# KevinLADLee/RoboRTS-Edu-SLAM

Measured on AMD Instinct MI355X. Metric: candidate-pose scorings/sec (1081-beam scan, 2000×2000 grid) at 1/2/4/8 GPUs, higher is better.
Workload: dtype f64; 1 GPU; config2: 1081-beam scans vs 2000x2000 @5cm fp32 grid, full 3-level coarse->fine->super-fine (sim-YAML windows 5070+1331+189 candidates/scan); levels=headline, scans_per_gpu=4096, parallelism=replicas x1 (scan-sharded, no collective)

## Files before the change

roborts-edu-slam_amd/csrc/csm_api.cpp:

```cpp
#include "csm_source_digest.h"
#include "csm_host.hpp"
#include "libm_sincos.hpp"

using namespace csmh;

extern "C" {

int csm_abi_version(void) { return CSM_ABI_VERSION; }

const char* csm_build_digest(void) { return CSM_SOURCE_DIGEST; }

int csm_create(int device, csm_ctx** out) {
  const char* lr = std::getenv("LOCAL_RANK");
  const char* lw = std::getenv("LOCAL_WORLD_SIZE");
  const int world = lw ? std::max(1, std::atoi(lw)) : 1;
  const int rank = (lr && world > 1) ? std::min(std::max(0, std::atoi(lr)), world - 1) : 0;
  return create_context(device, rank, world, out);
}

int csm_get_host_plan(csm_ctx* c, csm_host_plan* out) {
  if (!c || !out) return CSM_ERR_INVALID_ARG;
  *out = c->host_plan;
  return CSM_OK;
}
// ... 20 lines not shown
  if (const char* env = std::getenv("CSM_HOST_THREADS")) {
    const int v = std::atoi(env);
    if (v > 0) c->host_plan.threads = v;
  }
  c->host_threads = c->host_plan.threads;
  if (const char* env = std::getenv("CSM_FIRST_WINDOWS")) c->first_windows = c->first_windows_submit = std::max(0, std::atoi(env));
  if (const char* env = std::getenv("CSM_FIRST_WINDOWS_SUBMIT")) c->first_windows_submit = std::max(0, std::atoi(env));
  if (const char* env = std::getenv("CSM_SPLIT_HANDOFF_MIN")) c->split_handoff_min = std::max(2, std::atoi(env));
  if (const char* env = std::getenv("CSM_DEFER_HANDOFF")) c->defer_last_handoff = std::atoi(env) != 0;
  if (const char* env = std::getenv("CSM_HOST_SIGNAL")) c->host_signal = std::atoi(env) != 0;
  if (const char* env = std::getenv("CSM_FINISH")) {
    c->device_finish = std::strcmp(env, "host") != 0;
    c->fast_finish = std::strcmp(env, "exact") != 0;
  }
  if (const char* env = std::getenv("CSM_KERNEL")) {
    c->row_kernel = std::strcmp(env, "v2") != 0;
    c->box_kernel = std::strcmp(env, "v6") == 0 || std::strcmp(env, "v7") == 0;
    c->box_kernel = c->box_kernel || std::strcmp(env, "v8") == 0;
    c->phase_kernel = std::strcmp(env, "v7") == 0 || std::strcmp(env, "v8") == 0;
    c->tiny_kernel = std::strcmp(env, "v8") == 0;
    c->pair_kernel = false;
  }
  if (const char* env = std::getenv("CSM_PHASE_STRIPS")) c->phase_strips = std::atoi(env) != 0;
  if (const char* env = std::getenv("CSM_PHASE_MARGIN_LOG2"))
    c->phase_margin_log2 = std::max(2, std::min(std::atoi(env), 20));
  if (const char* env = std::getenv("CSM_PIPELINE")) {
    const int v = std::atoi(env);
    c->pipeline_min = v > 0 ? v : INT32_MAX;
  }
  if (const char* env = std::getenv("CSM_PIPELINE_PARTS"))
    c->pipeline_parts = std::max(2, std::min(std::atoi(env), csm_ctx::kMaxParts));
  if (const char* env = std::getenv("CSM_SKIP_DEAD_LISTS")) c->skip_dead_lists = std::atoi(env) != 0;
  if (const char* env = std::getenv("CSM_SMALL")) c->small_path = std::atoi(env) != 0;
  if (const char* env = std::getenv("CSM_LIST_REDUCE_MIN")) c->list_reduce_min = std::max<long long>(0, std::atoll(env));
  if (const char* env = std::getenv("CSM_STATS_DUMP")) c->stats_dump = std::atoi(env) != 0;
  if (const char* env = std::getenv("CSM_SCORE_MARKER")) c->score_marker = std::atoi(env) != 0;
  if (const char* env = std::getenv("CSM_DEVICE_TRIG")) c->device_trig = std::atoi(env) != 0;
#ifdef CSM_DEBUG_FIN
  c->debug_fin = true;
#endif
  if (c->each_slot([](LaunchSlot& s) { return s.create_sync_events(); }) != hipSuccess ||
      c->ev_pts.create(hipEventDisableTiming) != hipSuccess || c->ev_pack.create(hipEventDisableTiming) != hipSuccess ||
      c->x_stream.create(hipStreamNonBlocking) != hipSuccess) {
    delete c;
    return CSM_ERR_HIP;
  }
// ... 269 lines not shown
```

roborts-edu-slam_amd/csrc/csm_box.hip:

```cpp
#include <hip/hip_runtime.h>

#include <cstdint>
#include <cstdlib>

#include "csm_internal.hpp"
#include "csm_score_sink.hpp"

namespace csm {
namespace {

typedef int32_t v4i __attribute__((ext_vector_type(4)));

constexpr double kBoxMargin = 0x1p-20;

#ifndef CSM_RUN_SEG
#define CSM_RUN_SEG 1152
#endif
constexpr int kRunSeg = CSM_RUN_SEG;
#ifndef CSM_BOX_PF
#define CSM_BOX_PF 6
#endif
constexpr int kPF = CSM_BOX_PF;
#ifndef CSM_PAIR_ILP
#define CSM_PAIR_ILP 1
// ... 25 lines not shown
    const double tx = lx + hx;
    const double ty = ly + hy;
    const double fx = __builtin_amdgcn_fract(tx);
    const double fy = __builtin_amdgcn_fract(ty);
    const bool clean = tx >= 0.0 && ty >= 0.0 && fx >= kBoxMargin && fx <= 1.0 - kBoxMargin &&
                       fy >= kBoxMargin && fy <= 1.0 - kBoxMargin;
    const double lim = (double)(pad - nspan) - kBoxMargin;
    far = nspan > 0 && (tx <= lim || ty <= lim);
    ix0 = clean ? (int)tx : 0;
    iy0 = clean ? (int)ty : 0;
    return clean;
  }
  template <bool STRIP = false>
  __device__ __forceinline__ int offsets(const double2 p, int cb, uint64_t& slow) const {
    double lx, ly;
    int ix0, iy0;
    bool far;
    const bool clean = box_test(p, lx, ly, ix0, iy0, far);
    const bool live = cb + lane < n_used;
    const uint64_t rej = __builtin_amdgcn_ballot_w64(live && !clean && !far);
    if (rej) slow |= 1ull << min(cb >> 6, 63);
    int o;
    if (STRIP) {
      constexpr int S = kStripShift, LS = S == 4 ? 2 : 0;
      const int c = (-(ix0 >> LS)) & (kStripCopies - 1);
      const int xs = (ix0 & ~(S - 1)) + S * c;
      o = (int)(__umul24((uint32_t)c, (uint32_t)copy_bytes >> 4) << 4) +
          (int)__umul24((uint32_t)(xs >> 4), (uint32_t)strip_bytes) + iy0 * 16 + (ix0 & (S - 1));
    } else {
      o = iy0 * pitch4 + (ix0 << cell_shift);
    }
    return (live && clean && ix0 < sx + pad && iy0 < sy + pad) ? o : zero_off;
  }
  __device__ __forceinline__ double2 point(int cb) const {
    const uint32_t i = (uint32_t)min(cb + lane, n_used - 1);
    return *reinterpret_cast<const double2*>(reinterpret_cast<const char*>(P) + __umul24(i, step16));
  }

  template <int PF = kPF, typename CT = int32_t, bool STRIP = false, bool ILP = false>
  __device__ __forceinline__ int build_runs(int s0, int s1, int32_t* run_off, CT* run_cnt, int scratch,
                                            uint64_t& slow) const {
    int nruns = 0;
    double2 pq[PF];
#pragma unroll
    for (int u = 0; u < PF; ++u) {
      pq[u] = point(s0 + 64 * u);
      __builtin_amdgcn_sched_barrier(0);
    }
    for (int cb0 = s0; cb0 < s1; cb0 += 64 * PF) {
      int offv[PF];
      if constexpr (ILP) {
// ... 199 lines not shown
#ifdef CSM_BOX_TRACE
constexpr int kBoxTraceWaves = 4096;
__device__ unsigned long long g_box_trace[kBoxTraceWaves][12];
__device__ int g_box_trace_n;
#define BOX_STAMP() ((unsigned long long)__builtin_amdgcn_s_memtime())
#endif

constexpr int kPairPD = 2;
#ifndef CSM_PAIR_SEG
#define CSM_PAIR_SEG 576
#endif
constexpr int kPairSeg = CSM_PAIR_SEG;
static_assert(kPairSeg % 64 == 0 && (kPairSeg + 128) * 4 >= 16 * 16 * 8,
              "whole 64-beam chunks; the sums' transpose (16 x 16 int64) reuses the run list");

#ifndef CSM_PAIR_WAVES
#define CSM_PAIR_WAVES 0
#endif
#if CSM_PAIR_WAVES > 0
#define CSM_PAIR_BOUNDS __launch_bounds__(64, CSM_PAIR_WAVES)
#else
#define CSM_PAIR_BOUNDS __launch_bounds__(64)
#endif
template <int B>
__device__ __forceinline__ uint32_t byte_x8(uint32_t w) {
  static_assert(B >= 0 && B < 4, "a byte of a dword");
  uint32_t r;
  if constexpr (B == 0)
    asm("v_lshlrev_b32_sdwa %0, 3, %1 dst_sel:DWORD dst_unused:UNUSED_PAD src0_sel:DWORD src1_sel:BYTE_0"
        : "=v"(r) : "v"(w));
  else if constexpr (B == 1)
    asm("v_lshlrev_b32_sdwa %0, 3, %1 dst_sel:DWORD dst_unused:UNUSED_PAD src0_sel:DWORD src1_sel:BYTE_1"
        : "=v"(r) : "v"(w));
  else if constexpr (B == 2)
    asm("v_lshlrev_b32_sdwa %0, 3, %1 dst_sel:DWORD dst_unused:UNUSED_PAD src0_sel:DWORD src1_sel:BYTE_2"
        : "=v"(r) : "v"(w));
  else
    asm("v_lshlrev_b32_sdwa %0, 3, %1 dst_sel:DWORD dst_unused:UNUSED_PAD src0_sel:DWORD src1_sel:BYTE_3"
        : "=v"(r) : "v"(w));
  return r;
}

constexpr int kPairNoRunBeams = 128;

template <int NS, bool BEST, bool NORUN = false>
__global__ CSM_PAIR_BOUNDS void score_box_pair_kernel(LevelWork L, const ScanWork* __restrict__ scans,
                                                            const double2* __restrict__ pts,
                                                            const AngleEntry* __restrict__ angles,
                                                            double* __restrict__ out,
                                                            BestPartial* __restrict__ partials) {
  static_assert(NS >= 1 && NS <= kPalMaxSpace, "corner phase (<= 3) + NS cells within one 16-byte row piece");
  static_assert(kPairPD == 2, "a slot's step: one ds_read_b128 of pair offsets, one u16 of counts");
#ifdef CSM_BOX_TRACE
  unsigned long long tr[12] = {BOX_STAMP(), 0, 0, 0, 0, 0, 0, 0, 0, 0, 0, 0};
  unsigned long long tq = 0;
#endif
  const int bid = dev::xcd_remap(blockIdx.x, gridDim.x);
  dev::clear_word(L);
  const int win = bid / L.n_angles;
  const int a = bid - win * L.n_angles;
  const ScanWork S = scans[win];
  const AngleEntry ae = angles[S.angle_off + a];
  const int lane = threadIdx.x;
  const int k = lane & 15, slot = lane >> 4;
// ... 300 lines not shown
```

roborts-edu-slam_amd/csrc/csm_device.hpp:

```cpp
#pragma once

#include <hip/hip_runtime.h>

#include "csm_internal.hpp"

namespace csm {
namespace dev {

__device__ __forceinline__ void clear_word(int32_t* word, int32_t tag) {
  if (word && blockIdx.x == 0 && threadIdx.x == 0)
    __hip_atomic_store(reinterpret_cast<uint64_t*>(word), (uint64_t)(uint32_t)tag << 32, __ATOMIC_RELAXED,
                       __HIP_MEMORY_SCOPE_AGENT);
}
__device__ __forceinline__ void clear_word(const LevelWork& L) { clear_word(L.clear_word, L.clear_tag); }

__device__ __forceinline__ int xcd_remap(int orig, int nwg) {
  const int xcd = orig & 7;
  const int q = nwg >> 3, r = nwg & 7;
  const int base = (xcd < r) ? xcd * (q + 1) : r * (q + 1) + (xcd - r) * q;
  return base + (orig >> 3);
}

__device__ __forceinline__ double penalized(const LevelWork& L, const ScanWork& S, double acc, double x,
                                           double y, double angle) {
// ... 14 lines not shown
    }
  }
  return score;
}

__device__ __forceinline__ bool better(double s, int64_t f, double bs, int64_t bf) {
  return (s > bs) || (s == bs && f < bf);
}

__device__ __forceinline__ __amdgpu_buffer_rsrc_t uniform_rsrc(const void* p, int bytes) {
  const uint32_t lo = __builtin_amdgcn_readfirstlane((uint32_t)(uintptr_t)p);
  const uint32_t hi = __builtin_amdgcn_readfirstlane((uint32_t)((uintptr_t)p >> 32));
  return __builtin_amdgcn_make_buffer_rsrc((void*)(((uint64_t)hi << 32) | lo), (short)0, bytes, 0x00020000);
}

__device__ __forceinline__ void buffer_load_lds16(__amdgpu_buffer_rsrc_t rsrc,
                                                  __attribute__((address_space(3))) int32_t* lds,
                                                  int voffset) {
#if defined(__HIP_DEVICE_COMPILE__)
  __builtin_amdgcn_raw_ptr_buffer_load_lds(rsrc, lds, 16, voffset, 0, 0, 0);
#endif
}

__device__ __forceinline__ double bcast_lane(double v, int l) {
  const uint64_t u = __builtin_bit_cast(uint64_t, v);
  const uint32_t lo = __builtin_amdgcn_readlane((uint32_t)u, l);
  const uint32_t hi = __builtin_amdgcn_readlane((uint32_t)(u >> 32), l);
  return __builtin_bit_cast(double, ((uint64_t)hi << 32) | lo);
}

template <bool ROWS32>
__device__ __forceinline__ uint64_t swap_sum_u64(uint64_t u) {
  const uint32_t lo = (uint32_t)u, hi = (uint32_t)(u >> 32);
  if constexpr (ROWS32) {
    const auto l = __builtin_amdgcn_permlane32_swap(lo, lo, false, false);
    const auto h = __builtin_amdgcn_permlane32_swap(hi, hi, false, false);
    return (((uint64_t)h[0] << 32) | l[0]) + (((uint64_t)h[1] << 32) | l[1]);
  } else {
    const auto l = __builtin_amdgcn_permlane16_swap(lo, lo, false, false);
    const auto h = __builtin_amdgcn_permlane16_swap(hi, hi, false, false);
    return (((uint64_t)h[0] << 32) | l[0]) + (((uint64_t)h[1] << 32) | l[1]);
  }
}
template <int CTRL>
__device__ __forceinline__ uint64_t dpp_u64(uint64_t u) {
  const uint32_t lo = (uint32_t)__builtin_amdgcn_mov_dpp((int)(uint32_t)u, CTRL, 0xF, 0xF, false);
// ... 36 lines not shown
```

roborts-edu-slam_amd/csrc/csm_host.hpp:

```cpp
#pragma once

#include "csm.h"
#include "csm_internal.hpp"
#include "csm_finish_rules.hpp"
#include "csm_gridmap.h"
#include "csm_gridmap_internal.hpp"
#include "csm_resources.hpp"
#include "host_math.hpp"
#include "csm_pyramid.hpp"
#include "csm_search_match.hpp"
#include "csm_level_decision.hpp"

#include <algorithm>
#include <atomic>
#include <chrono>
#include <condition_variable>
#include <functional>
#include <memory>
#include <cfloat>
#include <cmath>
#include <cstdio>
#include <cstdlib>
#include <cstring>
#include <mutex>
// ... 355 lines not shown
  bool staging_dirty = false;
  csm_gridmap* reader_map = nullptr;
  csmh::HostBuf h_pts;
  csmh::Event ev_pts;
  bool ev_pts_used = false;
  bool host_signal = true;
  double t_call = 0.0, t_exit = 0.0;
  bool device_finish = true;
  bool fast_finish = true;
  int device_finish_min = 1;
  bool row_kernel = true;
  bool phase_kernel = true;
  bool tiny_kernel = true;
  int phase_margin_log2 = 20;
  csmh::DevBuf pal_grid, pal_vals, pal_scratch;
  csmh::DevBuf pal_strips;
  bool pal_strips_ok = false;
  bool pair_kernel = true;
  csmh::DevBuf istrips;
  uint64_t istrips_gen = 0;
  const int32_t* istrips_src = nullptr;
  bool istrips_ok = false;
  bool phase_strips = true;
  int32_t pal_n = 0;
  uint64_t pal_gen = 0;
  const int32_t* pal_src = nullptr;
  bool box_kernel = true;
  csmh::DevBuf split_slab, split_arrive, small_dev;
  csmh::HostBuf h_small_in, h_small_out;
  uint32_t flag_seq = 0;
  bool small_path = true;
  int small_max_windows = 32;
  int split_target_blocks = 512;
  int fast_wide_windows = 0;
  csmh::HostBuf h_pack;
  csmh::Event ev_pack;
  bool ev_pack_used = false;
  std::vector<double> pts_host;
  csmh::DevBuf d_updates;

  static constexpr int kParkedGrids = 3;
  csmh::GridState parked[kParkedGrids];
  uint64_t grid_clock = 0;
  void swap_grid(csmh::GridState& g) {
    std::swap(static_cast<csmh::GridState&>(*this), g);
    grid_gen = ++gen_clock;
// ... 235 lines not shown
```

roborts-edu-slam_amd/csrc/csm_launch.cpp:

```cpp
#include "csm_host.hpp"
#include "libm_sincos_table.hpp"

namespace csmh {

int window_dims(const csm_param& P, Dims& d) {
  if (!(P.search_angle_resolution > 0.0) || !(P.search_space_resolution > 0.0) ||
      !(P.search_angle_offset >= 0.0) || !(P.search_space_size >= 0.0))
    return CSM_ERR_INVALID_ARG;
  const double half = (P.search_angle_offset * 2) / 2;
  const double na = std::floor(half * 2 / P.search_angle_resolution) + 1;
  const double ns = round_half_away(P.search_space_size / P.search_space_resolution) + 1;
  if (!(na >= 1.0 && na < 1e7 && ns >= 1.0 && ns < 1e7)) return CSM_ERR_INVALID_ARG;
  d.n_angles = (int32_t)na;
  d.n_space = (int32_t)ns;
  d.n_cand = (int64_t)d.n_angles * d.n_space * d.n_space;
  return CSM_OK;
}

bool beam_rule(int n, int use_point_size, int& step, int& use, int& n_used) {
  use = use_point_size;
  if (n < 2 * use) {
    use = n;
    step = 1;
  } else {
// ... 391 lines not shown
constexpr bool kTailFinish = CSM_TAIL_FINISH != 0;

struct Launch {
  csm_ctx* c;
  const csm_param& P;
  const Dims& D;
  const Geometry& G;
  const std::vector<WindowPlan>& plans;
  const AngleEntry* angles;
  size_t n_angle_entries;
  Finish mode;
  int skip_lists;
  WinSpan sp;
  int nw, w0, w1;
  bool whole;
  double f;
  LevelSummary S{};
  LevelDecision dec{};
  LaunchShape shape{};
  csm::PhaseTable PT{};
  bool sig = false;
  int64_t stride = 0;
  LevelWork L{};
  csm::FinishArgs SA{};
  csm::FinishOut* sig_out = nullptr;
  int32_t* d_done = nullptr;
  const int32_t* flags_h = nullptr;
  int n_flags = 0;
  hipStream_t done_stream = nullptr;
  int nr() const { return w1 - w0; }
  bool time_fin() const { return c->profiling && !c->profile_first_level; }
  int validate(), decide(), level_work(const std::vector<int64_t>& pt_offsets, const std::vector<int32_t>& grid_index);
  int stage_signalled(), stage_tail(), send_inputs(), scoring();
  int launch_finish_timed(const csm::FinishArgs& A, csm::FinishOut* out, hipStream_t fs, bool fast_done);
  int finish_scores_to_host(), finish_signalled(), finish_device(), finish_best(BestPartial* best_out);
  void fill_pending(const char* kname, PendingRun& p);
};

int Launch::validate() {
  if (!whole) {
    bool ok = mode == Finish::kDevice && (sp.score || sp.finish) && 0 <= w0 && w0 < w1 && w1 <= nw &&
              n_angle_entries == (size_t)nw * (size_t)D.n_angles && sp.level;
    for (int w = w0; ok && w < w1; ++w) ok = plans[(size_t)w].angle_off == (int64_t)w * D.n_angles;
    if (!ok) return c->fail(CSM_ERR_INVALID_ARG, "run_windows: bad window span");
  }
  const int st = ensure_int_grid(c);
// ... 18 lines not shown
  K.int_grid = c->int_ok;
  K.tail_finish = kTailFinish && sig;
  K.box = c->box_kernel && f == 1.0 && csm::box_supported(D.n_space) && pad_ok;
  K.phase = use_int && c->phase_kernel && f < 1.0 && phase_table(f, D.n_space, c->phase_margin_log2, PT) &&
            csm::phase_supported(D.n_space, PT.cells, PT.nq) && pad_ok;
  K.tiny = c->tiny_kernel && f < 1.0 && csm::tiny_supported(D.n_space, f) && pad_ok && gridi_cells * 4 < INT32_MAX;
  dec = level_decide(S, K, w0, w1);
  if (!dec.valid) return c->fail(CSM_ERR_INVALID_ARG, "run_windows: bad window span");
  ShapeFacts F;
  F.best = mode == Finish::kBest;
  if (use_int && c->row_kernel && D.n_space <= 64) {
    const double span = (double)(D.n_space - 1) * f;
    F.rows_sq = csm::rows_pick_sq(D.n_space, (int)std::floor(span * (1.0 + 1e-9) + 1e-9) + 2);
    if (c->info.size_x < 4 * F.rows_sq) F.rows_sq = 0;
  }
  int st;
  if (dec.box && c->pair_kernel && csm::box_pair_supported(D.n_space)) {
    if ((st = ensure_palette(c)) != CSM_OK) return st;
    F.pair_ok = c->pal_n > 0 && gridi_cells <= INT32_MAX && c->pal_strips_ok;
  }
  const int64_t tile_n = (D.n_space + 15) / 16;
  F.tiled_ok = c->box_kernel && f == 1.0 && pad_ok && (int64_t)nw * tile_n * tile_n * D.n_angles <= INT32_MAX;
  if (dec.phase && c->phase_strips && (st = ensure_istrips(c)) != CSM_OK) return st;
  shape = launch_shape(dec, D.n_angles, D.n_space, F);
  if (shape.bps * nr() > INT32_MAX) return c->fail(CSM_ERR_UNSUPPORTED, "window too large for one launch");
  stride = score_stride(c, D, mode);
  return CSM_OK;
}

int Launch::level_work(const std::vector<int64_t>& pt_offsets, const std::vector<int32_t>& grid_index) {
  const hipError_t e = c->h_sw.ensure((size_t)nw * sizeof(ScanWork));
  if (e != hipSuccess) return c->hip_fail(e, "hipHostMalloc(scans)");
  ScanWork* sw = (ScanWork*)c->h_sw.p;
  if (sp.score && !(sp.sw_ready && sp.sw_stride == stride && (const void*)sp.sw_ready == (const void*)sw))
    fill_scan_work(D, plans, pt_offsets, grid_index, sw, (size_t)w0, (size_t)w1, stride);
  L = make_level_work(c, P, D, G, nr(), dec.use_int);
  const bool tiled = shape.kernel == ScoreKernel::kBoxTiled;
  L.blocks_per_scan = tiled ? D.n_angles : (int32_t)shape.bps;
  L.max_n_used = dec.max_n_used;
  L.tile_n = tiled ? shape.ktiles : 0;
  if (shape.kernel == ScoreKernel::kBoxPair) {
    const csm::StripGeom SG = csm::strip_geom(c->info.size_x, c->info.size_y);
    L.pal_n = c->pal_n;
    L.pal_grid = (const uint8_t*)c->pal_grid.p;
    L.pal_vals = (const int32_t*)c->pal_vals.p;
    L.pal_stride = (int64_t)c->pitch * (c->info.size_y + csm::kGridiPadRows);
    L.pal_strips = (const uint8_t*)c->pal_strips.p;
    L.strip_bytes = (int32_t)SG.strip_bytes;
    L.strip_copy_bytes = (int32_t)SG.copy_bytes;
    L.strip_grid_bytes = SG.grid_bytes;
  }
  if (shape.kernel == ScoreKernel::kPhase && c->phase_strips && c->istrips_ok) {
    const csm::StripGeom SG = csm::istrip_geom(c->info.size_x, c->info.size_y);
    L.istrips = (const int32_t*)c->istrips.p;
    L.istrip_bytes = (int32_t)SG.strip_bytes;
    L.istrip_copy_bytes = (int32_t)SG.copy_bytes;
    L.istrip_grid_bytes = SG.grid_bytes;
  }
  L.n_cols = (int32_t)shape.n_cols;
  L.ktiles = shape.ktiles;
  L.col_blocks = (int32_t)shape.col_blocks;
  return CSM_OK;
}

// ... 252 lines not shown
    if (fst != CSM_OK) return fst;
  }
  const double tp1 = c->profiling ? now_ms() : 0.0;
  if (c->profiling) c->account("host:launch:flush_events", (float)(tp1 - tp0), 0.0, 0.0);
  int st;
  hipError_t e;
  if ((st = X.validate()) != CSM_OK) return st;
  if (X.whole && mode != Finish::kBest && c->int_ok && X.S.in_range && small_launch(c, D, nw))
    return run_windows_small(c, P, D, G, plans, pt_offsets, angles, n_angle_entries, grid_index,
                             mode == Finish::kDevice, pend, skip_lists);
  if ((st = X.decide()) != CSM_OK) return st;
  if ((st = X.level_work(pt_offsets, grid_index)) != CSM_OK) return st;
  if (X.sig && (st = X.stage_signalled()) != CSM_OK) return st;
  if (X.dec.tail && (st = X.stage_tail()) != CSM_OK) return st;
  if ((e = c->scans.ensure((size_t)nw * sizeof(ScanWork))) != hipSuccess) return c->hip_fail(e, "hipMalloc(scans)");
  if ((e = c->angles.ensure(n_angle_entries * sizeof(AngleEntry))) != hipSuccess) return c->hip_fail(e, "hipMalloc(angles)");
  const double tl0 = c->profiling ? now_ms() : 0.0;
  if (c->profiling) c->account("host:launch:prep", (float)(tl0 - tp1), 0.0, 0.0);
  if (sp.score && (st = X.send_inputs()) != CSM_OK) return st;
  char kname[48];
  score_kernel_name(X.shape, kname, sizeof(kname));
  const double tl1 = c->profiling ? now_ms() : 0.0;
  if ((st = X.scoring()) != CSM_OK) return st;
  if (c->profiling && mode != Finish::kBest) {
    c->account("host:launch:inputs", (float)(tl1 - tl0), 0.0, 0.0);
    c->account("host:launch:score", (float)(now_ms() - tl1), 0.0, 0.0);
  }
  if (!sp.finish) return CSM_OK;
  const double tl2 = (c->profiling && mode != Finish::kBest) ? now_ms() : 0.0;
  X.done_stream = c->d2h;
  st = mode == Finish::kBest ? X.finish_best(best_out)
       : mode == Finish::kScoresToHost ? X.finish_scores_to_host()
       : X.sig ? X.finish_signalled()
               : X.finish_device();
  if (st != CSM_OK) return st;
  PendingRun local;
  PendingRun& p = pend ? *pend : local;
  X.fill_pending(kname, p);
  if ((e = hipEventRecord(c->ev_done, X.done_stream)) != hipSuccess) return c->hip_fail(e, "hipEventRecord");
  if (c->profiling && tl2 > 0.0) c->account("host:launch:finish", (float)(now_ms() - tl2), 0.0, 0.0);
  if (c->profiling && X.sig) {
    char nm[48];
    std::snprintf(nm, sizeof(nm), "finish:%s<%lld>", X.dec.tail ? "fused" : "separate", (long long)D.n_cand);
    c->account(nm, 0.f, 0.0, (double)nw);
  }
  return pend ? CSM_OK : wait_run(c, p);
// ... 122 lines not shown
```

roborts-edu-slam_amd/csrc/csm_phase.hip:

```cpp
#include <hip/hip_runtime.h>

#include <cstdint>

#include "csm_internal.hpp"
#include "csm_score_sink.hpp"

namespace csm {
namespace {

#ifndef CSM_PHASE_SEG
#define CSM_PHASE_SEG 576
#endif
constexpr int kSeg = CSM_PHASE_SEG;
constexpr int kEntG = 31;
static_assert(kEntG * ((1LL << 26) - 1) < 2147483647LL, "a lane's int32 partial");
constexpr int kChunks = kSeg / 64;
#ifndef CSM_PHASE_DEPTH
#define CSM_PHASE_DEPTH 4
#endif
constexpr int kD = CSM_PHASE_DEPTH;
static_assert(kD <= 32, "int32 partial sums fold every kD groups");
static_assert((kD & (kD - 1)) == 0, "CSM_PHASE_DEPTH must be a power of two");
static_assert(kSeg % 64 == 0, "CSM_PHASE_SEG must be whole 64-beam chunks");

typedef int32_t v4i __attribute__((ext_vector_type(4)));

#ifndef CSM_PHASE_WAVES
#define CSM_PHASE_WAVES 4
#endif

constexpr int kPhaseShortBeams = 128;

template <int NS, int C, int NQ, bool BEST, bool ST, int KCH = kChunks>
__global__ __launch_bounds__(64, CSM_PHASE_WAVES) void score_phase_kernel(LevelWork L, PhaseTable T,
                                                         const ScanWork* __restrict__ scans,
                                                         const double2* __restrict__ pts,
                                                         const AngleEntry* __restrict__ angles,
                                                         double* __restrict__ out,
                                                         BestPartial* __restrict__ partials) {
  constexpr int NP = NQ * NQ;
  constexpr int NPC = (C + 3) / 4;
  constexpr int LPS = C * NPC;
  constexpr int SL = 64 / LPS;
  constexpr int PC = C * C;
  static_assert(LPS <= 64 && NP <= 64 && NS <= kPhaseMaxSpace && NQ <= kPhaseMaxBuckets, "layout");
  static_assert(2 * NP + 1 < 256, "group tags are bytes");
  constexpr int kList = 64 * KCH + NP * (SL - 1) + 3 * SL * kD + 64;
  constexpr int kMaxGroups = kList / SL + 1;
  __shared__ int32_t list[kList];
  __shared__ int32_t cursor[NP];
  __shared__ int32_t ngroups_s;
  __shared__ uint8_t gtag[kMaxGroups];
  __shared__ __attribute__((aligned(16))) int64_t psum[(NP + 1) * PC];
  static_assert(sizeof(psum) >= tail::kBytesA + tail::kBytesB, "the fused finish's LDS (csm_tail.hpp)");
  __shared__ int8_t oxs[NQ][kPhaseMaxSpace];

  const int bid = dev::xcd_remap(blockIdx.x, gridDim.x);
  dev::clear_word(L);
  const int win = bid / L.n_angles;
  const int a = bid - win * L.n_angles;
  const ScanWork S = scans[win];
  const AngleEntry ae = angles[S.angle_off + a];
  const int lane = threadIdx.x;
  const bool cact = lane < SL * LPS;
  const int slot = cact ? lane / LPS : 0;
  const int within = cact ? lane - slot * LPS : 0;
  const int cv = within / NPC;
  const int ch = within - cv * NPC;
  const double f = L.step_cells;
  const double x_0 = S.x0 + 0 * f;
  const double y_0 = S.y0 + 0 * f;
  const int sx = L.size_x, sy = L.size_y;
  const int pitch4 = L.pitch * 4;
  constexpr int kRowB = kIStripCells * 4;
  static_assert(!ST || 4 * NPC <= kIStripCells + 4, "a box row's pieces stay within its strip row and the next");
  constexpr int kPad = ST ? kIStripPadLo : 0;
  const int zero_off = ST ? (kPad + sy) * kRowB : sy * pitch4;
  const double2* __restrict__ P = pts + S.pts_off;
  const int step = S.step;
  const int n_used = S.n_used;
  const int32_t* gi = L.gridi + (int64_t)S.grid_index * L.gridi_stride;
  const int32_t* gsrc = ST ? L.istrips + (int64_t)S.grid_index * (L.istrip_grid_bytes / 4) : gi;
  const __amdgpu_buffer_rsrc_t rsrc =
      dev::uniform_rsrc(gsrc, ST ? (int)L.istrip_grid_bytes : (int)(L.gridi_stride * 4));
  const int voff = ST ? cv * kRowB + ch * 16 : cv * pitch4 + ch * 16;

  for (int i = lane; i < NQ * kPhaseMaxSpace; i += 64) oxs[i / kPhaseMaxSpace][i % kPhaseMaxSpace] =
      T.ox[i / kPhaseMaxSpace][i % kPhaseMaxSpace];
  for (int i = lane; i < (NP + 1) * PC; i += 64) psum[i] = 0;

  auto bucket = [&](double ph, bool& ok) -> int {
    int q = 0;
    bool hit = false;
#pragma unroll
    for (int b = 0; b < NQ; ++b) {
      const bool in = b < T.nq && ph >= T.lo[b] && ph <= T.hi[b];
      q = in ? b : q;
      hit |= in;
    }
    ok = ok && hit;
    return q;
  };
  auto classify = [&](const double2 p, int cb, int lim, double& lx, double& ly, bool& rejected) -> int2 {
    lx = ae.cosine * p.x - ae.sine * p.y;
    ly = ae.sine * p.x + ae.cosine * p.y;
    const double tx = (lx + x_0) + (0.5 + kPad);
    const double ty = (ly + y_0) + (0.5 + kPad);
    bool ok = tx >= 0.0 && ty >= 0.0;
    const double fx = __builtin_amdgcn_fract(tx);
    const double fy = __builtin_amdgcn_fract(ty);
    int qx, qy;
    if (T.uniform) {
      const double nqd = (double)T.nq;
      const double sx_ = fx * nqd, sy_ = fy * nqd;
      const double rx = __builtin_amdgcn_fract(sx_), ry = __builtin_amdgcn_fract(sy_);
      qx = (int)(sx_ - rx);
      qy = (int)(sy_ - ry);
      ok = ok && rx >= T.ulo && rx <= T.uhi && ry >= T.ulo && ry <= T.uhi && qx < T.nq && qy < T.nq;
    } else {
      qx = bucket(fx, ok);
      qy = bucket(fy, ok);
    }
    const bool live = cb + lane < lim;
    const double lim_far = kPad - 1.0 - (NS - 1) * f - 0x1p-20;
    const bool far = tx <= lim_far || ty <= lim_far;
    rejected = live && !ok && !far;
    const int ix0 = ok ? (int)tx : 0;
    const int iy0 = ok ? (int)ty : 0;
    const bool use = live && ok && ix0 < sx + kPad && iy0 < sy + kPad;
    int o;
    if (ST) {
      const int c = (ix0 >> 2) & 1;
      const int xs = (ix0 & ~3) + 4 * c;
      o = c * L.istrip_copy_bytes + (xs >> 3) * L.istrip_bytes + iy0 * kRowB + (ix0 & 3) * 4;
    } else {
      o = iy0 * pitch4 + ix0 * 4;
    }
    return make_int2(use ? o : 0, use ? qx * NQ + qy : -1);
  };
  auto point = [&](int b) { return P[(int64_t)min(b, n_used - 1) * step]; };

  constexpr int NC = NS * NS;
  constexpr int R = (NC + 63) / 64;
  __syncthreads();
  uint32_t oxj[R], oyk[R];
#pragma unroll
  for (int r = 0; r < R; ++r) {
    const int t = lane + 64 * r;
    const int j = t < NC ? t / NS : 0;
    const int k = t < NC ? t - j * NS : 0;
    oxj[r] = 0;
    oyk[r] = 0;
#pragma unroll
    for (int q = 0; q < NQ; ++q) {
// ... 10 lines not shown
  static_assert(KCH >= 1 && KCH <= kChunks, "segments of at most kSeg beams");
  for (int s0 = 0; s0 < n_used; s0 += 64 * KCH) {
    const int s1 = min(n_used, s0 + 64 * KCH);
    double2 pq[KCH];
#pragma unroll
    for (int u = 0; u < KCH; ++u) pq[u] = point(s0 + 64 * u + lane);
    if (lane < NP) cursor[lane] = 0;
    __syncthreads();
    int offr[KCH], pairr[KCH];
#pragma unroll
    for (int u = 0; u < KCH; ++u) {
      const int cb = s0 + 64 * u;
      double lx, ly;
      bool rej;
      const int2 c = classify(pq[u], cb, s1, lx, ly, rej);
      slow |= (uint64_t)(__builtin_amdgcn_ballot_w64(rej) != 0) << min(cb >> 6, 63);
      offr[u] = c.x;
      pairr[u] = c.y;
      if (c.y >= 0) atomicAdd(&cursor[c.y], 1);
    }
    __syncthreads();
    {
      const int cnt = lane < NP ? cursor[lane] : 0;
      const int g = (cnt + SL - 1) / SL;
      int gi_ = g;
#pragma unroll
      for (int o = 1; o < 64; o <<= 1) {
        const int tg = __shfl_up(gi_, o, 64);
        if (lane >= o) gi_ += tg;
      }
      const int g0p = gi_ - g;
      if (lane < NP) {
        cursor[lane] = g0p * SL;
        for (int k = 0; k < g; ++k) gtag[g0p + k] = (uint8_t)(2 * lane + ((k / kEntG) & 1));
      }
      if (lane == NP - 1) ngroups_s = gi_;
    }
    __syncthreads();
    const int ngroups = __builtin_amdgcn_readfirstlane(ngroups_s);
    const int ng_pad = (ngroups + kD - 1) / kD * kD;
    for (int i = lane; i < (ng_pad + 2 * kD) * SL; i += 64) list[i] = zero_off;
    for (int i = ngroups + lane; i < ng_pad + kD; i += 64) gtag[i] = (uint8_t)(2 * NP);
    __syncthreads();
#pragma unroll
    for (int u = 0; u < KCH; ++u)
      if (pairr[u] >= 0) list[atomicAdd(&cursor[pairr[u]], 1)] = offr[u];
    __syncthreads();
    if (ngroups > 0) {
      v4i buf[kD];
#pragma unroll
      for (int j = 0; j < kD; ++j) {
        buf[j] = __builtin_amdgcn_raw_buffer_load_b128(rsrc, list[j * SL + slot] + voff, 0, 0);
        __builtin_amdgcn_sched_barrier(0);
      }
      int32_t part[4] = {0, 0, 0, 0};
      int t_prev = __builtin_amdgcn_readfirstlane((int)gtag[0]);
      auto flush = [&](int tag) {
        int64_t* dst = psum + (tag >> 1) * PC + lane_cell;
#pragma unroll
        for (int t = 0; t < 4; ++t) {
          if (cact && 4 * ch + t < C)
            __hip_atomic_fetch_add(dst + t, (int64_t)part[t], __ATOMIC_RELAXED, __HIP_MEMORY_SCOPE_WORKGROUP);
// ... 74 lines not shown
#pragma unroll
          for (int r = 0; r < R; ++r) sum[r] += v[u][r];
      }
    }
  }

  dev::ScoreSink<BEST> sink;
#pragma unroll
  for (int r = 0; r < R; ++r) {
    const int t = lane + 64 * r;
    if (t < NC) {
      const int j = t / NS, k = t - (t / NS) * NS;
      const double accd = dev::fixed_point_acc(L, sum[r], n_used);
      const double xj = S.x0 + j * f;
      const double yk = S.y0 + k * f;
      sink.add(L, S, out, ((int64_t)a * NS + j) * NS + k, dev::penalized(L, S, accd, xj, yk, ae.angle));
    }
  }
  if (!BEST && L.tail.on) __syncthreads();
  sink.done(L, S, angles, out, a, partials + (int64_t)win * L.blocks_per_scan + a, reinterpret_cast<char*>(psum),
            reinterpret_cast<char*>(psum) + tail::kBytesA);
}

template <int NS, int C, int NQ, bool ST, int KCH>
hipError_t launch_phase_k(const LevelWork& L, const PhaseTable& T, const ScanWork* s, const double2* p,
                          const AngleEntry* an, double* out, BestPartial* part, unsigned nblk, hipStream_t stream) {
  if (part)
    hipLaunchKernelGGL((score_phase_kernel<NS, C, NQ, true, ST, KCH>), dim3(nblk), dim3(64), 0, stream, L, T, s, p,
                       an, out, part);
  else
    hipLaunchKernelGGL((score_phase_kernel<NS, C, NQ, false, ST, KCH>), dim3(nblk), dim3(64), 0, stream, L, T, s, p,
                       an, out, part);
  return hipGetLastError();
}

template <int NS, int C, int NQ, bool ST>
hipError_t launch_phase(const LevelWork& L, const PhaseTable& T, const ScanWork* s, const double2* p,
                        const AngleEntry* an, double* out, BestPartial* part, unsigned nblk, hipStream_t stream) {
  if (L.max_n_used > 0 && L.max_n_used <= kPhaseShortBeams)
    return launch_phase_k<NS, C, NQ, ST, kPhaseShortBeams / 64>(L, T, s, p, an, out, part, nblk, stream);
  return launch_phase_k<NS, C, NQ, ST, kChunks>(L, T, s, p, an, out, part, nblk, stream);
}

}

bool phase_supported(int ns, int cells, int nq) { return ns == 11 && cells == 5 && nq == 5; }

hipError_t launch_score_phase(const LevelWork& L, const PhaseTable& T, const ScanWork* d_scans, const double* d_pts,
                              const AngleEntry* d_angles, double* d_out, BestPartial* d_partials, int ns,
                              hipStream_t stream) {
  const int64_t nblk = (int64_t)L.n_scans * L.n_angles;
  if (nblk <= 0 || nblk > INT32_MAX || !L.int_mode || !(L.step_cells < 1.0) || L.blocks_per_scan != L.n_angles ||
      L.pitch < L.size_x + kGridiPadCols || L.pitch % 4 != 0 || !phase_supported(ns, T.cells, T.nq) ||
      T.cells > kGridiPadCols + 1)
    return hipErrorInvalidValue;
  for (int q = 0; q < T.nq; ++q)
    for (int j = 0; j < ns; ++j)
      if (T.ox[q][j] < 0 || T.ox[q][j] >= T.cells) return hipErrorInvalidValue;
  const double2* p = reinterpret_cast<const double2*>(d_pts);
  if (L.istrips) {
    const StripGeom G = istrip_geom(L.size_x, L.size_y);
    if (L.istrip_bytes != G.strip_bytes || L.istrip_copy_bytes != G.copy_bytes || L.istrip_grid_bytes != G.grid_bytes ||
        G.grid_bytes > INT32_MAX)
      return hipErrorInvalidValue;
    return launch_phase<11, 5, 5, true>(L, T, d_scans, p, d_angles, d_out, d_partials, (unsigned)nblk, stream);
  }
  return launch_phase<11, 5, 5, false>(L, T, d_scans, p, d_angles, d_out, d_partials, (unsigned)nblk, stream);
}

}
```

Baseline: 13.28 billion scorings/s.

## Add palette-indexed byte-strip variant of the phase scoring kernel

Adds a PAL variant of the phase kernel that reads the grid as palette-indexed byte strips instead of int32 strips. It loads 8-byte pieces for two beams at once and combines their palette indices into a lookup into a shared table of pairwise sums. The aim is to shrink gather bytes per beam and halve the number of accumulations. It is gated on the pair kernel and palette availability, and it adds new list and tag bookkeeping plus double-precision accumulation that is converted back to fixed point.

```diff
diff --git a/roborts-edu-slam_amd/csrc/csm_api.cpp b/roborts-edu-slam_amd/csrc/csm_api.cpp
--- a/roborts-edu-slam_amd/csrc/csm_api.cpp
+++ b/roborts-edu-slam_amd/csrc/csm_api.cpp
@@ -66,6 +66,7 @@
     c->pair_kernel = false;
   }
   if (const char* env = std::getenv("CSM_PHASE_STRIPS")) c->phase_strips = std::atoi(env) != 0;
+  if (const char* env = std::getenv("CSM_PHASE_PAL")) c->phase_pal = std::atoi(env) != 0;
   if (const char* env = std::getenv("CSM_PHASE_MARGIN_LOG2"))
     c->phase_margin_log2 = std::max(2, std::min(std::atoi(env), 20));
   if (const char* env = std::getenv("CSM_PIPELINE")) {
diff --git a/roborts-edu-slam_amd/csrc/csm_box.hip b/roborts-edu-slam_amd/csrc/csm_box.hip
--- a/roborts-edu-slam_amd/csrc/csm_box.hip
+++ b/roborts-edu-slam_amd/csrc/csm_box.hip
@@ -71,11 +71,7 @@
     if (rej) slow |= 1ull << min(cb >> 6, 63);
     int o;
     if (STRIP) {
-      constexpr int S = kStripShift, LS = S == 4 ? 2 : 0;
-      const int c = (-(ix0 >> LS)) & (kStripCopies - 1);
-      const int xs = (ix0 & ~(S - 1)) + S * c;
-      o = (int)(__umul24((uint32_t)c, (uint32_t)copy_bytes >> 4) << 4) +
-          (int)__umul24((uint32_t)(xs >> 4), (uint32_t)strip_bytes) + iy0 * 16 + (ix0 & (S - 1));
+      o = dev::pal_strip_offset(ix0, iy0, strip_bytes, copy_bytes);
     } else {
       o = iy0 * pitch4 + (ix0 << cell_shift);
     }
@@ -321,24 +317,7 @@
 #else
 #define CSM_PAIR_BOUNDS __launch_bounds__(64)
 #endif
-template <int B>
-__device__ __forceinline__ uint32_t byte_x8(uint32_t w) {
-  static_assert(B >= 0 && B < 4, "a byte of a dword");
-  uint32_t r;
-  if constexpr (B == 0)
-    asm("v_lshlrev_b32_sdwa %0, 3, %1 dst_sel:DWORD dst_unused:UNUSED_PAD src0_sel:DWORD src1_sel:BYTE_0"
-        : "=v"(r) : "v"(w));
-  else if constexpr (B == 1)
-    asm("v_lshlrev_b32_sdwa %0, 3, %1 dst_sel:DWORD dst_unused:UNUSED_PAD src0_sel:DWORD src1_sel:BYTE_1"
-        : "=v"(r) : "v"(w));
-  else if constexpr (B == 2)
-    asm("v_lshlrev_b32_sdwa %0, 3, %1 dst_sel:DWORD dst_unused:UNUSED_PAD src0_sel:DWORD src1_sel:BYTE_2"
-        : "=v"(r) : "v"(w));
-  else
-    asm("v_lshlrev_b32_sdwa %0, 3, %1 dst_sel:DWORD dst_unused:UNUSED_PAD src0_sel:DWORD src1_sel:BYTE_3"
-        : "=v"(r) : "v"(w));
-  return r;
-}
+using dev::byte_x8;
 
 constexpr int kPairNoRunBeams = 128;
 
diff --git a/roborts-edu-slam_amd/csrc/csm_device.hpp b/roborts-edu-slam_amd/csrc/csm_device.hpp
--- a/roborts-edu-slam_amd/csrc/csm_device.hpp
+++ b/roborts-edu-slam_amd/csrc/csm_device.hpp
@@ -60,6 +60,34 @@
 #endif
 }
 
+__device__ __forceinline__ int pal_strip_offset(int ix0, int iy0, int strip_bytes, int copy_bytes) {
+  constexpr int S = kStripShift, LS = S == 4 ? 2 : 0;
+  const int c = (-(ix0 >> LS)) & (kStripCopies - 1);
+  const int xs = (ix0 & ~(S - 1)) + S * c;
+  return (int)(__umul24((uint32_t)c, (uint32_t)copy_bytes >> 4) << 4) +
+         (int)__umul24((uint32_t)(xs >> 4), (uint32_t)strip_bytes) + iy0 * 16 + (ix0 & (S - 1));
+}
+constexpr int kStripMaxPhase = kStripShift - 1;
+
+template <int B>
+__device__ __forceinline__ uint32_t byte_x8(uint32_t w) {
+  static_assert(B >= 0 && B < 4, "a byte of a dword");
+  uint32_t r;
+  if constexpr (B == 0)
+    asm("v_lshlrev_b32_sdwa %0, 3, %1 dst_sel:DWORD dst_unused:UNUSED_PAD src0_sel:DWORD src1_sel:BYTE_0"
+        : "=v"(r) : "v"(w));
+  else if constexpr (B == 1)
+    asm("v_lshlrev_b32_sdwa %0, 3, %1 dst_sel:DWORD dst_unused:UNUSED_PAD src0_sel:DWORD src1_sel:BYTE_1"
+        : "=v"(r) : "v"(w));
+  else if constexpr (B == 2)
+    asm("v_lshlrev_b32_sdwa %0, 3, %1 dst_sel:DWORD dst_unused:UNUSED_PAD src0_sel:DWORD src1_sel:BYTE_2"
+        : "=v"(r) : "v"(w));
+  else
+    asm("v_lshlrev_b32_sdwa %0, 3, %1 dst_sel:DWORD dst_unused:UNUSED_PAD src0_sel:DWORD src1_sel:BYTE_3"
+        : "=v"(r) : "v"(w));
+  return r;
+}
+
 __device__ __forceinline__ double bcast_lane(double v, int l) {
   const uint64_t u = __builtin_bit_cast(uint64_t, v);
   const uint32_t lo = __builtin_amdgcn_readlane((uint32_t)u, l);
diff --git a/roborts-edu-slam_amd/csrc/csm_host.hpp b/roborts-edu-slam_amd/csrc/csm_host.hpp
--- a/roborts-edu-slam_amd/csrc/csm_host.hpp
+++ b/roborts-edu-slam_amd/csrc/csm_host.hpp
@@ -401,6 +401,7 @@
   const int32_t* istrips_src = nullptr;
   bool istrips_ok = false;
   bool phase_strips = true;
+  bool phase_pal = true;
   int32_t pal_n = 0;
   uint64_t pal_gen = 0;
   const int32_t* pal_src = nullptr;
diff --git a/roborts-edu-slam_amd/csrc/csm_launch.cpp b/roborts-edu-slam_amd/csrc/csm_launch.cpp
--- a/roborts-edu-slam_amd/csrc/csm_launch.cpp
+++ b/roborts-edu-slam_amd/csrc/csm_launch.cpp
@@ -437,6 +437,7 @@
   bool sig = false;
   int64_t stride = 0;
   LevelWork L{};
+  bool phase_pal = false;
   csm::FinishArgs SA{};
   csm::FinishOut* sig_out = nullptr;
   int32_t* d_done = nullptr;
@@ -501,6 +502,7 @@
   const int64_t tile_n = (D.n_space + 15) / 16;
   F.tiled_ok = c->box_kernel && f == 1.0 && pad_ok && (int64_t)nw * tile_n * tile_n * D.n_angles <= INT32_MAX;
   if (dec.phase && c->phase_strips && (st = ensure_istrips(c)) != CSM_OK) return st;
+  if (dec.phase && c->phase_pal && c->pair_kernel && (st = ensure_palette(c)) != CSM_OK) return st;
   shape = launch_shape(dec, D.n_angles, D.n_space, F);
   if (shape.bps * nr() > INT32_MAX) return c->fail(CSM_ERR_UNSUPPORTED, "window too large for one launch");
   stride = score_stride(c, D, mode);
@@ -518,7 +520,10 @@
   L.blocks_per_scan = tiled ? D.n_angles : (int32_t)shape.bps;
   L.max_n_used = dec.max_n_used;
   L.tile_n = tiled ? shape.ktiles : 0;
-  if (shape.kernel == ScoreKernel::kBoxPair) {
+  const int64_t gridi_cells = (int64_t)c->pitch * (c->info.size_y + csm::kGridiPadRows);
+  phase_pal = shape.kernel == ScoreKernel::kPhase && c->phase_pal && c->pair_kernel && c->pal_n > 0 &&
+              c->pal_n <= csm::kPairMaxPal && gridi_cells <= INT32_MAX && c->pal_strips_ok;
+  if (shape.kernel == ScoreKernel::kBoxPair || phase_pal) {
     const csm::StripGeom SG = csm::strip_geom(c->info.size_x, c->info.size_y);
     L.pal_n = c->pal_n;
     L.pal_grid = (const uint8_t*)c->pal_grid.p;
@@ -817,6 +822,8 @@
   score_kernel_name(X.shape, kname, sizeof(kname));
   const double tl1 = c->profiling ? now_ms() : 0.0;
   if ((st = X.scoring()) != CSM_OK) return st;
+  if (c->profiling && sp.score && w0 == 0 && X.shape.kernel == ScoreKernel::kPhase)
+    c->account(X.phase_pal ? "phase:pal" : "phase:int", 0.f, 0.0, (double)nw);
   if (c->profiling && mode != Finish::kBest) {
     c->account("host:launch:inputs", (float)(tl1 - tl0), 0.0, 0.0);
     c->account("host:launch:score", (float)(now_ms() - tl1), 0.0, 0.0);
diff --git a/roborts-edu-slam_amd/csrc/csm_phase.hip b/roborts-edu-slam_amd/csrc/csm_phase.hip
--- a/roborts-edu-slam_amd/csrc/csm_phase.hip
+++ b/roborts-edu-slam_amd/csrc/csm_phase.hip
@@ -31,7 +31,10 @@
 
 constexpr int kPhaseShortBeams = 128;
 
-template <int NS, int C, int NQ, bool BEST, bool ST, int KCH = kChunks>
+constexpr int kPalSlots = 12;
+constexpr int kPalPD = 2;
+
+template <int NS, int C, int NQ, bool BEST, bool ST, int KCH = kChunks, bool PAL = false>
 __global__ __launch_bounds__(64, CSM_PHASE_WAVES) void score_phase_kernel(LevelWork L, PhaseTable T,
                                                          const ScanWork* __restrict__ scans,
                                                          const double2* __restrict__ pts,
@@ -39,19 +42,22 @@
                                                          double* __restrict__ out,
                                                          BestPartial* __restrict__ partials) {
   constexpr int NP = NQ * NQ;
-  constexpr int NPC = (C + 3) / 4;
+  constexpr int NPC = PAL ? 1 : (C + 3) / 4;
   constexpr int LPS = C * NPC;
   constexpr int SL = 64 / LPS;
+  static_assert(!PAL || (ST && SL == kPalSlots), "palette form: 12 pair slots of C rows, strip coordinates");
   constexpr int PC = C * C;
   static_assert(LPS <= 64 && NP <= 64 && NS <= kPhaseMaxSpace && NQ <= kPhaseMaxBuckets, "layout");
   static_assert(2 * NP + 1 < 256, "group tags are bytes");
-  constexpr int kList = 64 * KCH + NP * (SL - 1) + 3 * SL * kD + 64;
-  constexpr int kMaxGroups = kList / SL + 1;
-  __shared__ int32_t list[kList];
+  constexpr int kPalSteps = (((64 * KCH + NP) / 2 + kPalSlots - 1) / kPalSlots + kPalPD - 1) / kPalPD * kPalPD;
+  constexpr int kPalEntries = kPalSlots * kPalSteps + kPalPD;
+  constexpr int kList = PAL ? 2 * kPalEntries : 64 * KCH + NP * (SL - 1) + 3 * SL * kD + 64;
+  constexpr int kMaxGroups = PAL ? kPalEntries : kList / SL + 1;
+  __shared__ __attribute__((aligned(8))) int32_t list[kList];
   __shared__ int32_t cursor[NP];
   __shared__ int32_t ngroups_s;
   __shared__ uint8_t gtag[kMaxGroups];
-  __shared__ __attribute__((aligned(16))) int64_t psum[(NP + 1) * PC];
+  __shared__ __attribute__((aligned(16))) int64_t psum[(NP + (PAL ? 0 : 1)) * PC];
   static_assert(sizeof(psum) >= tail::kBytesA + tail::kBytesB, "the fused finish's LDS (csm_tail.hpp)");
   __shared__ int8_t oxs[NQ][kPhaseMaxSpace];
 
@@ -74,20 +80,34 @@
   const int pitch4 = L.pitch * 4;
   constexpr int kRowB = kIStripCells * 4;
   static_assert(!ST || 4 * NPC <= kIStripCells + 4, "a box row's pieces stay within its strip row and the next");
-  constexpr int kPad = ST ? kIStripPadLo : 0;
-  const int zero_off = ST ? (kPad + sy) * kRowB : sy * pitch4;
+  constexpr int kPad = PAL ? kStripPadLo : ST ? kIStripPadLo : 0;
+  static_assert(!PAL || (kStripPadLo >= NS && kStripPadLo == kIStripPadLo), "palette strips' low padding");
+  static_assert(!PAL || (dev::kStripMaxPhase + C <= 8 && C <= kStripPadRows), "corner phase + C cells in 8 bytes");
+  const int zero_off = PAL ? (kPad + sy) * 16 : ST ? (kPad + sy) * kRowB : sy * pitch4;
   const double2* __restrict__ P = pts + S.pts_off;
   const int step = S.step;
   const int n_used = S.n_used;
   const int32_t* gi = L.gridi + (int64_t)S.grid_index * L.gridi_stride;
-  const int32_t* gsrc = ST ? L.istrips + (int64_t)S.grid_index * (L.istrip_grid_bytes / 4) : gi;
-  const __amdgpu_buffer_rsrc_t rsrc =
-      dev::uniform_rsrc(gsrc, ST ? (int)L.istrip_grid_bytes : (int)(L.gridi_stride * 4));
-  const int voff = ST ? cv * kRowB + ch * 16 : cv * pitch4 + ch * 16;
+  const void* gsrc = PAL  ? (const void*)(L.pal_strips + (int64_t)S.grid_index * L.strip_grid_bytes)
+                     : ST ? (const void*)(L.istrips + (int64_t)S.grid_index * (L.istrip_grid_bytes / 4))
+                          : (const void*)gi;
+  const __amdgpu_buffer_rsrc_t rsrc = dev::uniform_rsrc(
+      gsrc, PAL ? (int)L.strip_grid_bytes : ST ? (int)L.istrip_grid_bytes : (int)(L.gridi_stride * 4));
+  const int voff = PAL ? cv * 16 : ST ? cv * kRowB + ch * 16 : cv * pitch4 + ch * 16;
+  const int sh = L.pal_n <= 8 ? 3 : 4;
+  double* tab = nullptr;
+  if constexpr (PAL) {
+    __shared__ double tab_s[256];
+    tab = tab_s;
+    for (int i = lane; i < 256; i += 64) {
+      const int ia = i & ((1 << sh) - 1), ib = i >> sh;
+      tab[i] = (ia < L.pal_n && ib < L.pal_n) ? (double)L.pal_vals[ia] + (double)L.pal_vals[ib] : 0.0;
+    }
+  }
 
   for (int i = lane; i < NQ * kPhaseMaxSpace; i += 64) oxs[i / kPhaseMaxSpace][i % kPhaseMaxSpace] =
       T.ox[i / kPhaseMaxSpace][i % kPhaseMaxSpace];
-  for (int i = lane; i < (NP + 1) * PC; i += 64) psum[i] = 0;
+  for (int i = lane; i < (int)(sizeof(psum) / sizeof(psum[0])); i += 64) psum[i] = 0;
 
   auto bucket = [&](double ph, bool& ok) -> int {
     int q = 0;
@@ -129,7 +149,9 @@
     const int iy0 = ok ? (int)ty : 0;
     const bool use = live && ok && ix0 < sx + kPad && iy0 < sy + kPad;
     int o;
-    if (ST) {
+    if (PAL) {
+      o = dev::pal_strip_offset(ix0, iy0, L.strip_bytes, L.strip_copy_bytes);
+    } else if (ST) {
       const int c = (ix0 >> 2) & 1;
       const int xs = (ix0 & ~3) + 4 * c;
       o = c * L.istrip_copy_bytes + (xs >> 3) * L.istrip_bytes + iy0 * kRowB + (ix0 & 3) * 4;
@@ -186,7 +208,7 @@
     __syncthreads();
     {
       const int cnt = lane < NP ? cursor[lane] : 0;
-      const int g = (cnt + SL - 1) / SL;
+      const int g = PAL ? (cnt + 1) >> 1 : (cnt + SL - 1) / SL;
       int gi_ = g;
 #pragma unroll
       for (int o = 1; o < 64; o <<= 1) {
@@ -195,13 +217,107 @@
       }
       const int g0p = gi_ - g;
       if (lane < NP) {
-        cursor[lane] = g0p * SL;
-        for (int k = 0; k < g; ++k) gtag[g0p + k] = (uint8_t)(2 * lane + ((k / kEntG) & 1));
+        cursor[lane] = g0p * (PAL ? 2 : SL);
+        for (int k = 0; k < g; ++k) gtag[g0p + k] = PAL ? (uint8_t)lane : (uint8_t)(2 * lane + ((k / kEntG) & 1));
       }
       if (lane == NP - 1) ngroups_s = gi_;
     }
     __syncthreads();
     const int ngroups = __builtin_amdgcn_readfirstlane(ngroups_s);
+    if constexpr (PAL) {
+      const int K = ((ngroups + kPalSlots - 1) / kPalSlots + kPalPD - 1) / kPalPD * kPalPD;
+      const int n_ent = kPalSlots * K + kPalPD;
+      for (int i = lane; i < 2 * n_ent; i += 64) list[i] = zero_off;
+      for (int i = ngroups + lane; i < n_ent; i += 64) gtag[i] = (uint8_t)NP;
+      __syncthreads();
+#pragma unroll
+      for (int u = 0; u < KCH; ++u)
+        if (pairr[u] >= 0) list[atomicAdd(&cursor[pairr[u]], 1)] = offr[u];
+      __syncthreads();
+      if (ngroups > 0) {
+        typedef int32_t v2i __attribute__((ext_vector_type(2)));
+        constexpr int kPieceMask = kStripShift == 1 ? ~0 : ~15;
+        auto load = [&](int off) -> v2i {
+          return __builtin_amdgcn_raw_buffer_load_b64(rsrc, (off & kPieceMask) + voff, 0, 0);
+        };
+        const int e0 = slot * K;
+        const int2* lp = reinterpret_cast<const int2*>(list) + e0;
+        const uint8_t* tp = gtag + e0;
+        double acc[C];
+#pragma unroll
+        for (int c = 0; c < C; ++c) acc[c] = 0.0;
+        auto flush = [&](int tag) {
+          if (cact && tag < NP) {
+            int64_t* dst = psum + tag * PC + cv * C;
+#pragma unroll
+            for (int c = 0; c < C; ++c) {
+              const int64_t v = __builtin_bit_cast(int64_t, acc[c] + 0x1.8p52) - __builtin_bit_cast(int64_t, 0x1.8p52);
+              __hip_atomic_fetch_add(dst + c, v, __ATOMIC_RELAXED, __HIP_MEMORY_SCOPE_WORKGROUP);
+            }
+          }
+#pragma unroll
+          for (int c = 0; c < C; ++c) acc[c] = 0.0;
+        };
+        int2 ocur[kPalPD];
+        int tcur[kPalPD];
+        v2i dA[kPalPD], dB[kPalPD];
+#pragma unroll
+        for (int j = 0; j < kPalPD; ++j) {
+          ocur[j] = lp[j];
+          tcur[j] = tp[j];
+          dA[j] = load(ocur[j].x);
+          dB[j] = load(ocur[j].y);
+          __builtin_amdgcn_sched_barrier(0);
+        }
+        int t_prev = tcur[0];
+        const char* tb = reinterpret_cast<const char*>(tab);
+        for (int i0 = 0; i0 < K; i0 += kPalPD) {
+          int2 onext[kPalPD];
+          int tnext[kPalPD];
+#pragma unroll
+          for (int j = 0; j < kPalPD; ++j) {
+            onext[j] = lp[i0 + kPalPD + j];
+            tnext[j] = tp[i0 + kPalPD + j];
+          }
+#pragma unroll
+          for (int j = 0; j < kPalPD; ++j) {
+            if (tcur[j] != t_prev) flush(t_prev);
+            t_prev = tcur[j];
+            const v2i xa = dA[j], xb = dB[j];
+            uint32_t w0, w1;
+            if constexpr (kStripShift == 1) {
+              w0 = (uint32_t)xa.x | ((uint32_t)xb.x << sh);
+              w1 = (uint32_t)xa.y | ((uint32_t)xb.y << sh);
+            } else {
+              const uint32_t sa = (uint32_t)ocur[j].x & 3u, sb = (uint32_t)ocur[j].y & 3u;
+              w0 = __builtin_amdgcn_alignbyte((uint32_t)xa.y, (uint32_t)xa.x, sa) |
+                   (__builtin_amdgcn_alignbyte((uint32_t)xb.y, (uint32_t)xb.x, sb) << sh);
+              w1 = __builtin_amdgcn_alignbyte(0u, (uint32_t)xa.y, sa) |
+                   (__builtin_amdgcn_alignbyte(0u, (uint32_t)xb.y, sb) << sh);
+            }
+            dA[j] = load(onext[j].x);
+            dB[j] = load(onext[j].y);
+#pragma unroll
+            for (int c = 0; c < C; ++c) {
+              const uint32_t wc = c < 4 ? w0 : w1;
+              const uint32_t o = (c & 3) == 0 ? dev::byte_x8<0>(wc) : (c & 3) == 1 ? dev::byte_x8<1>(wc)
+                               : (c & 3) == 2 ? dev::byte_x8<2>(wc) : dev::byte_x8<3>(wc);
+              acc[c] += *reinterpret_cast<const double*>(tb + o);
+            }
+            __builtin_amdgcn_sched_barrier(0);
+          }
+#pragma unroll
+          for (int j = 0; j < kPalPD; ++j) {
+            ocur[j] = onext[j];
+            tcur[j] = tnext[j];
+          }
+        }
+        flush(t_prev);
+        asm volatile("s_waitcnt vmcnt(0)" ::: "memory");
+      }
+      __syncthreads();
+      continue;
+    }
     const int ng_pad = (ngroups + kD - 1) / kD * kD;
     for (int i = lane; i < (ng_pad + 2 * kD) * SL; i += 64) list[i] = zero_off;
     for (int i = ngroups + lane; i < ng_pad + kD; i += 64) gtag[i] = (uint8_t)(2 * NP);
@@ -322,24 +438,24 @@
             reinterpret_cast<char*>(psum) + tail::kBytesA);
 }
 
-template <int NS, int C, int NQ, bool ST, int KCH>
+template <int NS, int C, int NQ, bool ST, int KCH, bool PAL>
 hipError_t launch_phase_k(const LevelWork& L, const PhaseTable& T, const ScanWork* s, const double2* p,
                           const AngleEntry* an, double* out, BestPartial* part, unsigned nblk, hipStream_t stream) {
   if (part)
-    hipLaunchKernelGGL((score_phase_kernel<NS, C, NQ, true, ST, KCH>), dim3(nblk), dim3(64), 0, stream, L, T, s, p,
+    hipLaunchKernelGGL((score_phase_kernel<NS, C, NQ, true, ST, KCH, PAL>), dim3(nblk), dim3(64), 0, stream, L, T, s, p,
                        an, out, part);
   else
-    hipLaunchKernelGGL((score_phase_kernel<NS, C, NQ, false, ST, KCH>), dim3(nblk), dim3(64), 0, stream, L, T, s, p,
+    hipLaunchKernelGGL((score_phase_kernel<NS, C, NQ, false, ST, KCH, PAL>), dim3(nblk), dim3(64), 0, stream, L, T, s, p,
                        an, out, part);
   return hipGetLastError();
 }
 
-template <int NS, int C, int NQ, bool ST>
+template <int NS, int C, int NQ, bool ST, bool PAL = false>
 hipError_t launch_phase(const LevelWork& L, const PhaseTable& T, const ScanWork* s, const double2* p,
                         const AngleEntry* an, double* out, BestPartial* part, unsigned nblk, hipStream_t stream) {
   if (L.max_n_used > 0 && L.max_n_used <= kPhaseShortBeams)
-    return launch_phase_k<NS, C, NQ, ST, kPhaseShortBeams / 64>(L, T, s, p, an, out, part, nblk, stream);
-  return launch_phase_k<NS, C, NQ, ST, kChunks>(L, T, s, p, an, out, part, nblk, stream);
+    return launch_phase_k<NS, C, NQ, ST, kPhaseShortBeams / 64, PAL>(L, T, s, p, an, out, part, nblk, stream);
+  return launch_phase_k<NS, C, NQ, ST, kChunks, PAL>(L, T, s, p, an, out, part, nblk, stream);
 }
 
 }
@@ -358,6 +474,14 @@
     for (int j = 0; j < ns; ++j)
       if (T.ox[q][j] < 0 || T.ox[q][j] >= T.cells) return hipErrorInvalidValue;
   const double2* p = reinterpret_cast<const double2*>(d_pts);
+  if (L.pal_strips) {
+    const StripGeom G = strip_geom(L.size_x, L.size_y);
+    if (L.pal_n < 1 || L.pal_n > kPairMaxPal || !L.pal_vals || L.strip_bytes != G.strip_bytes ||
+        L.strip_copy_bytes != G.copy_bytes || L.strip_grid_bytes != G.grid_bytes || G.grid_bytes > INT32_MAX ||
+        (int64_t)L.size_y * 16 > INT32_MAX)
+      return hipErrorInvalidValue;
+    return launch_phase<11, 5, 5, true, true>(L, T, d_scans, p, d_angles, d_out, d_partials, (unsigned)nblk, stream);
+  }
   if (L.istrips) {
     const StripGeom G = istrip_geom(L.size_x, L.size_y);
     if (L.istrip_bytes != G.strip_bytes || L.istrip_copy_bytes != G.copy_bytes || L.istrip_grid_bytes != G.grid_bytes ||
```

Measured after the change: 13.65 billion scorings/s, median of 6. 2.8% higher.
